# OmerMersin/video-stab

Hardware: AMD Instinct MI355X
Metric: stabilized frames/sec @1080p (whole job; warp-stage HBM GB/s in roofline) (higher is better)
Workload: dtype u8

## Files before the change

video-stab_amd/csrc/batch_schedule.cpp:

```cpp
#include <cstring>
#include <new>

#include "stab_internal.h"

using namespace vsd;

struct vs_batch {
    int device = 0, S = 0, B = 0, cap = 0;
    bool own = false;
    std::vector<vs_stab*> m;
    vs_stab* ref = nullptr;
    std::string err;
    FirstFailure failure;
    hipStream_t st = nullptr, st_pre = nullptr, st_det = nullptr, st_up = nullptr;
    bool allocated = false;
    uint8_t* h_tables = nullptr;
    size_t h_set_bytes = 0, ho_pairs = 0, ho_lk = 0, ho_rs = 0, ho_tail = 0, ho_gf = 0, ho_seg = 0;
    uint8_t* d_all = nullptr;
    uint8_t *d_lk[2] = {nullptr, nullptr}, *d_rs[2] = {nullptr, nullptr}, *d_tail[2] = {nullptr, nullptr}, *d_seg[2] = {nullptr, nullptr}, *d_gf = nullptr;
    uint8_t* d_tin[2] = {nullptr, nullptr};
    ImgPair* d_pairs[2] = {nullptr, nullptr};
    size_t up_bytes = 0;
    int pre_rel_step = -1;
    double* d_MinvB[2] = {nullptr, nullptr};
// ... 186 lines not shown

int fill_stream_items(vs_batch* g, vs_stab* s, const vs_batch::HostSet& H, const BorderPlan& bp, int ndue, int first, StepPlan& P) {
    const vs_params_c& p = s->p;
    const int ns = (int)s->bq.size(), dset = g->dev_set(P.k), set = g->pend_set;
    vs_batch::Ready& R = g->next;
    int npad = 0;
    for (int i = 0; i < ns; i++) {
        const int idx = first + i;
        const vs_stab::BFrame& b = s->bq[i];
        const vs_stab::ItemBufs& it = s->items[i];
        LKLevel L[MAX_PYR];
        fill_lk_levels(s, b.pv, b.c, L);
        const int cap = std::max(b.lk_cap, 0);
        P.n_max = std::max(P.n_max, cap);
        uint8_t *rs = H.rs + ransac_item_bytes() * idx, *tail = H.tail + tail_item_bytes() * idx;
        VS_OBJ_TRY(g, lk_fill_item(H.lk + lk_item_bytes() * idx, L, s->levels, s->d_pts[b.lk_buf], cap, s->d_npts[b.lk_buf], it.next, it.status, it.err,
                              p.lk_win_size, p.lk_max_iters, p.lk_epsilon));
        VS_OBJ_TRY(g, ransac_fill_item(rs, s->d_pts[b.lk_buf], it.next, it.status, cap, s->d_npts[b.lk_buf], it.vp, it.vc, it.m, 4, p.ransac_threshold,
                                  p.ransac_max_iters, s->tab, it.counts, it.model, it.inliers, it.info, s->d_traj, &s->tp, s->d_dbg, b.have_prev_gray));
        ransac_item_set_last(rs, i == ns - 1 ? 1 : 0);
        ransac_item_set_tail_in(rs, g->d_tin[dset] + tail_in_bytes() * idx);
        double* minv = nullptr;
        WarpTabJob jobs[2] = {{nullptr, nullptr, nullptr, 0, 0}, {nullptr, nullptr, nullptr, 0, 0}};
        if (b.out_due) {
            const int j = P.npend++;
            minv = g->d_MinvB[set] + 12 * j;
            R.srcs[j] = b.out_frame; R.dsts[j] = b.d_out; R.slots[j] = b.out_slot; R.owner[j] = s; R.pad_idx[j] = npad;
            if (P.all_apart && std::min(WARP_BATCH_MAX, ndue - j / WARP_BATCH_MAX * WARP_BATCH_MAX) >= WARP_TAB_MIN) {
                const WarpEnds e = warp_ends(s, b.out_frame, b.d_out, npad, bp);
                int32_t* T = g->d_tabs[set] + (size_t)j * g->tab_ints;
                jobs[0] = WarpTabJob{T, e.src, e.dst, bp.pw, bp.ph};
// ... 118 lines not shown
    g->last_det_batch = k;
    return VS_OK;
}

int step_issue_main(vs_batch* g, const std::vector<vs_stab*>& act, const StepPlan& P, bool warps_go, int kd) {
    const vs_stab* s0 = g->ref;
    const int dset = g->dev_set(P.k), set = g->pend_set;
    hipStream_t st = g->st;
    if (warps_go && g->last_warp_set >= 0) VS_OBJ_HIP(g, hipStreamWaitEvent(st, g->ev_warp[g->last_warp_set], 0));
    else VS_OBJ_HIP(g, hipStreamWaitEvent(st, g->ev_bpre, 0));
    for (vs_stab* s : act)
        if (s->pts_pending[0]) { VS_OBJ_HIP(g, hipStreamWaitEvent(st, s->pts_event[0], 0)); s->pts_pending[0] = false; }
    if (kd >= 0) VS_OBJ_HIP(g, hipStreamWaitEvent(st, g->det_event(kd), 0));
    {
        StageScope t(g->ref, VS_STAGE_LK, st);
        VS_OBJ_TRY(g, launch_pyr_lk_batch(g->d_lk[dset], P.n, P.n_max, s0->p.lk_win_size, st));
    }
    {
        StageScope t(g->ref, VS_STAGE_RANSAC, st);
        VS_OBJ_TRY(g, launch_ransac_score_batch(g->d_rs[dset], P.n, s0->p.ransac_max_iters, P.n_max, st));
    }
    for (vs_stab* s : act)
        if (s->dbg_delay_us > 0) { VS_OBJ_TRY(g, launch_spin(s->dbg_delay_us, st)); break; }
    if (P.npend > 0 && g->warp_valid[set]) {
        VS_OBJ_HIP(g, hipStreamWaitEvent(st, g->ev_warp[set], 0));
        g->warp_valid[set] = false;
    }
    {
        StageScope t(g->ref, VS_STAGE_TRAJ, st);
        VS_OBJ_TRY(g, launch_ransac_tail_group(g->d_rs[dset], g->d_tail[dset], g->d_seg[dset], g->d_tin[dset], P.nseg, P.max_n, P.n, P.any_apart, st));
    }
// ... 222 lines not shown
```

video-stab_amd/csrc/k_lk.hip:

```cpp
#include "vs_common.h"

namespace vsd {
namespace {

constexpr int MAX_LEVELS = 8;

struct LKArgs {
    LKLevel levels[MAX_LEVELS];
    int max_level;
    const float* prev_pts;
    float* next_pts;
    uint8_t* status;
    float* err;
    int n;
    const int32_t* d_n;
    int win;
    int max_count;
    double eps2;
};

template <int CTRL>
__device__ __forceinline__ int dpp_mov(int v) {
    return __builtin_amdgcn_update_dpp(0, v, CTRL, 0xF, 0xF, true);
}
// ... 30 lines not shown

__device__ __forceinline__ int descale(int x, int n) { return (x + (1 << (n - 1))) >> n; }

struct Weights { int w00, w01, w10, w11; };

__device__ __forceinline__ Weights make_weights(float a, float b) {
    Weights w;
    w.w00 = f_round((1.f - a) * (1.f - b) * 16384.f);
    w.w01 = f_round(a * (1.f - b) * 16384.f);
    w.w10 = f_round((1.f - a) * b * 16384.f);
    w.w11 = 16384 - w.w00 - w.w01 - w.w10;
    return w;
}

typedef const __attribute__((address_space(1))) uint8_t* gmem_u8;
__device__ __forceinline__ gmem_u8 uniform_global(const uint8_t* p) {
    const unsigned long long v = (unsigned long long)p;
    const unsigned lo = (unsigned)__builtin_amdgcn_readfirstlane((int)(unsigned)v), hi = (unsigned)__builtin_amdgcn_readfirstlane((int)(unsigned)(v >> 32));
    return (gmem_u8)(((unsigned long long)hi << 32) | lo);
}

constexpr int LK_MARGIN = 6;
constexpr int LK_WIN_MAX = 31;



__device__ __forceinline__ void divmod_small(int i, int d, float inv_d, int& q, int& r) {
    q = (int)(((float)i + 0.5f) * inv_d);
    r = i - q * d;
}

template <int NPX>
__device__ __forceinline__ void lk_track(const LKArgs& a, const int pt) {
    constexpr int WM = NPX <= 4 ? 16 : (NPX <= 7 ? 21 : LK_WIN_MAX);
    constexpr int PWM = WM + 1, RWM = WM + 1 + 2 * LK_MARGIN;
    constexpr int DR = NPX <= 7 ? 3 : 5;
    constexpr int PPM = (PWM + 2 + 3) & ~3;
    constexpr int SRM = (PWM + 1 + 3) / 4, NGM = (PWM + DR - 1) / DR;
    static_assert(SRM * NGM <= 64, "one derivative round per level");
    constexpr int PN = (PPM * (PWM + 2) + 63) / 64, RN = (RWM * RWM + 63) / 64;
    constexpr int PBYTES = (PN * 64 > PPM * (NGM * DR + 2) + 4 ? PN * 64 : PPM * (NGM * DR + 2) + 4);
    __shared__ __attribute__((aligned(16))) uint8_t pI_[4 + PBYTES];
    uint8_t* const pI = pI_ + 4;
    __shared__ __attribute__((aligned(16))) short2 pD[(PWM + 1) * PPM];
    __shared__ uint8_t region[RN * 64];
    const int lane = threadIdx.x;
    int n = a.n;
    if (a.d_n) { int dn = *a.d_n; n = dn < n ? dn : n; }
    if (pt >= n) return;
    const int win = a.win, area = win * win;
    const int PW = win + 1, PP = (PW + 2 + 3) & ~3;
    const int RW = win + 1 + 2 * LK_MARGIN;
    const float inv_pp = 1.0f / (float)PP, inv_rw = 1.0f / (float)RW, inv_win = 1.0f / (float)win;
    uint32_t off[NPX];
#pragma unroll
    for (int k = 0; k < NPX; k++) {
        const int p = lane + 64 * k;
        int yy = 0, xx = 0;
        if (p < area) divmod_small(p, win, inv_win, yy, xx);
        off[k] = (uint32_t)((yy + 1) * PP + xx + 1) | ((uint32_t)(yy * RW + xx) << 16);
    }
#define LK_VALID(k) (lane + 64 * (k) < area)
#define LK_POFF(k) ((int)(off[k] & 0xFFFFu))
#define LK_ROFF(k) ((int)(off[k] >> 16))
    int p_y0, p_x0, p_sy, p_sx, r_y0, r_x0, r_sy, r_sx;
    divmod_small(lane, PP, inv_pp, p_y0, p_x0);
    divmod_small(64, PP, inv_pp, p_sy, p_sx);
    divmod_small(lane, RW, inv_rw, r_y0, r_x0);
    divmod_small(64, RW, inv_rw, r_sy, r_sx);
    const float halfWin = (win - 1) * 0.5f;
    const float FLT_SCALE = 1.f / (1 << 20);
    const float px0 = a.prev_pts[2 * pt], py0 = a.prev_pts[2 * pt + 1];
    float outx = 0.f, outy = 0.f;
    int status = 1;
    float err = 0.f;

    for (int level = a.max_level; level >= 0; level--) {
        const LKLevel L = a.levels[level];
        const float scale = (float)(1. / (double)(1 << level));
        float prevx = px0 * scale, prevy = py0 * scale;
        if (level == a.max_level) { outx = prevx; outy = prevy; }
        else { outx = outx * 2.f; outy = outy * 2.f; }
        prevx -= halfWin; prevy -= halfWin;
        const int ipx = f_floor(prevx), ipy = f_floor(prevy);
        if (ipx < -win || ipx >= L.w || ipy < -win || ipy >= L.h) {
            if (level == 0) { status = 0; err = 0.f; }
            continue;
        }
        float cx = outx - halfWin, cy = outy - halfWin;
        int rx0 = f_floor(cx) - LK_MARGIN, ry0 = f_floor(cy) - LK_MARGIN;
        __syncthreads();
        const int pcount = PP * (PW + 2);
        if (ipx >= 1 && ipy >= 1 && ipx - 1 + PP <= L.w && ipy + PW + 1 <= L.h) {
            const gmem_u8 pbase = uniform_global(L.prev + ((size_t)(ipy - 1) * L.stride + (ipx - 1)));
            constexpr int PB_ = 10;
            int y = p_y0, x = p_x0;
#pragma unroll
            for (int k0 = 0; k0 < PN; k0 += PB_) {
                uint8_t vI[PB_];
#pragma unroll
                for (int k = k0; k < k0 + PB_ && k < PN; k++) {
                    const bool ok = lane + 64 * k < pcount;
                    vI[k - k0] = pbase[ok ? (uint32_t)(y * (int)L.stride + x) : 0u];
                    x += p_sx; y += p_sy;
                    if (x >= PP) { x -= PP; y++; }
                }
#pragma unroll
                for (int k = k0; k < k0 + PB_ && k < PN; k++) pI[lane + 64 * k] = vI[k - k0];
                __builtin_amdgcn_sched_barrier(0);
            }
        } else {
            int y = p_y0, x = p_x0;
            for (int i = lane; i < pcount; i += 64) {
                const int X = ipx - 1 + x, Y = ipy - 1 + y;
                pI[i] = L.prev[(size_t)reflect101(Y, L.h) * L.stride + reflect101(X, L.w)];
                x += p_sx; y += p_sy;
                if (x >= PP) { x -= PP; y++; }
            }
        }
        auto stage_region = [&]() {
            const bool inside = rx0 >= 0 && ry0 >= 0 && rx0 + RW <= L.w && ry0 + RW <= L.h;
            int y = r_y0, x = r_x0;
            asm volatile("" : "+v"(x), "+v"(y));
            if (inside) {
                const gmem_u8 rbase = uniform_global(L.next + ((size_t)ry0 * L.stride + rx0));
                constexpr int RB_ = 10;
#pragma unroll
                for (int k0 = 0; k0 < RN; k0 += RB_) {
                    uint8_t vR[RB_];
#pragma unroll
                    for (int k = k0; k < k0 + RB_ && k < RN; k++) {
                        const bool ok = lane + 64 * k < RW * RW;
                        vR[k - k0] = rbase[ok ? (uint32_t)(y * (int)L.stride + x) : 0u];
                        x += r_sx; y += r_sy;
                        if (x >= RW) { x -= RW; y++; }
                    }
#pragma unroll
                    for (int k = k0; k < k0 + RB_ && k < RN; k++) region[lane + 64 * k] = vR[k - k0];
                    __builtin_amdgcn_sched_barrier(0);
                }
            } else {
                for (int i = lane; i < RW * RW; i += 64) {
                    const int X = rx0 + x, Y = ry0 + y;
                    region[i] = L.next[(size_t)reflect101(Y, L.h) * L.stride + reflect101(X, L.w)];
                    x += r_sx; y += r_sy;
                    if (x >= RW) { x -= RW; y++; }
                }
            }
        };
        stage_region();
        __syncthreads();
        {
            const int sr = (PW + 1 + 3) >> 2;
            int g, c;
            divmod_small(lane, sr, 1.0f / (float)sr, g, c);
            const int y = 1 + g * DR, x = 4 * c;
            if (y <= PW) {
                const bool masked = !(ipx >= 0 && ipy >= 0 && ipx + PW <= L.w && ipy + PW <= L.h);
                int t[3][6];
                auto load_row = [&](int j, int* tj) {
                    const uint32_t* q = reinterpret_cast<const uint32_t*>(pI + j * PP) + c;
                    const uint32_t lo = q[-1], mid = q[0], hi = q[1];
                    tj[0] = lo >> 24;
                    tj[1] = mid & 255u; tj[2] = (mid >> 8) & 255u; tj[3] = (mid >> 16) & 255u; tj[4] = mid >> 24;
                    tj[5] = hi & 255u;
                };
                load_row(y - 1, t[0]);
                load_row(y, t[1]);
#pragma unroll
                for (int r = 0; r < DR; r++) {
                    const int* t0 = t[r % 3];
                    const int* t1 = t[(r + 1) % 3];
                    int* t2 = t[(r + 2) % 3];
                    load_row(y + r + 1, t2);
                    int av[6], bv[6];
#pragma unroll
                    for (int k = 0; k < 6; k++) {
                        av[k] = (t0[k] + t2[k]) * 3 + t1[k] * 10;
                        bv[k] = t2[k] - t0[k];
                    }
                    uint32_t o[4];
#pragma unroll
                    for (int k = 0; k < 4; k++) {
                        const int dx = av[k + 2] - av[k], dy = (bv[k + 2] + bv[k]) * 3 + bv[k + 1] * 10;
                        o[k] = ((uint32_t)dx & 0xFFFFu) | ((uint32_t)dy << 16);
                        if (masked && ((unsigned)(ipx - 1 + x + k) >= (unsigned)L.w || (unsigned)(ipy - 1 + y + r) >= (unsigned)L.h)) o[k] = 0u;
                    }
                    if (y + r <= PW) *reinterpret_cast<uint4*>(&pD[(y + r) * PP + x]) = make_uint4(o[0], o[1], o[2], o[3]);
                    __builtin_amdgcn_sched_barrier(0);
                }
            }
        }
        __syncthreads();
#pragma unroll
        for (int k = 0; k < NPX; k++) asm volatile("" : "+v"(off[k]));
        Weights wt = make_weights(prevx - ipx, prevy - ipy);
        short Iw[NPX], Ix[NPX], Iy[NPX];
        int pA11 = 0, pA12 = 0, pA22 = 0;
#pragma unroll
        for (int k = 0; k < NPX; k++) {
            const int o = LK_POFF(k);
            int ival = descale(__mul24((int)pI[o], wt.w00) + __mul24((int)pI[o + 1], wt.w01) +
                               __mul24((int)pI[o + PP], wt.w10) + __mul24((int)pI[o + PP + 1], wt.w11), 9);
            const short2 d00 = pD[o], d01 = pD[o + 1], d10 = pD[o + PP], d11 = pD[o + PP + 1];
            int ixval = descale(__mul24((int)d00.x, wt.w00) + __mul24((int)d01.x, wt.w01) +
                                __mul24((int)d10.x, wt.w10) + __mul24((int)d11.x, wt.w11), 14);
            int iyval = descale(__mul24((int)d00.y, wt.w00) + __mul24((int)d01.y, wt.w01) +
                                __mul24((int)d10.y, wt.w10) + __mul24((int)d11.y, wt.w11), 14);
            if (!LK_VALID(k)) { ival = 0; ixval = 0; iyval = 0; }
            Iw[k] = (short)ival; Ix[k] = (short)ixval; Iy[k] = (short)iyval;
            pA11 += __mul24(ixval, ixval);
            pA12 += __mul24(ixval, iyval);
            pA22 += __mul24(iyval, iyval);
        }
        const long long sA11 = wave_sum(pA11), sA12 = wave_sum(pA12), sA22 = wave_sum(pA22);
        const float A11 = (float)sA11 * FLT_SCALE, A12 = (float)sA12 * FLT_SCALE, A22 = (float)sA22 * FLT_SCALE;
// ... 11 lines not shown
            if (inx < -win || inx >= L.w || iny < -win || iny >= L.h) {
                if (level == 0) status = 0;
                break;
            }
            wt = make_weights(cx - inx, cy - iny);
            int lx = inx - rx0, ly = iny - ry0;
            if (!(lx >= 0 && ly >= 0 && lx + win + 1 <= RW && ly + win + 1 <= RW)) {
                __syncthreads();
                rx0 = inx - LK_MARGIN; ry0 = iny - LK_MARGIN;
                stage_region();
                __syncthreads();
                lx = LK_MARGIN; ly = LK_MARGIN;
            }
            int pb1 = 0, pb2 = 0;
            {
                const int rbase = ly * RW + lx;
#pragma unroll
                for (int k = 0; k < NPX; k++) {
                    const uint8_t* r0 = &region[rbase + LK_ROFF(k)];
                    const int v = descale(__mul24((int)r0[0], wt.w00) + __mul24((int)r0[1], wt.w01) +
                                          __mul24((int)r0[RW], wt.w10) + __mul24((int)r0[RW + 1], wt.w11), 9);
                    const int diff = v - Iw[k];
                    pb1 += __mul24(diff, (int)Ix[k]);
                    pb2 += __mul24(diff, (int)Iy[k]);
                }
            }
            const long long sb1 = wave_sum(pb1), sb2 = wave_sum(pb2);
            const float b1 = (float)sb1 * FLT_SCALE, b2 = (float)sb2 * FLT_SCALE;
            const float dx = (A12 * b2 - A22 * b1) * D;
            const float dy = (A12 * b1 - A11 * b2) * D;
            cx += dx; cy += dy;
            outx = cx + halfWin; outy = cy + halfWin;
            if ((double)dx * (double)dx + (double)dy * (double)dy <= a.eps2) break;
            if (j > 0 && (double)fabsf(dx + pdx) < 0.01 && (double)fabsf(dy + pdy) < 0.01) {
                outx -= dx * 0.5f; outy -= dy * 0.5f;
                break;
            }
            pdx = dx; pdy = dy;
        }
        if (status && level == 0) {
            const float npx = outx - halfWin, npy = outy - halfWin;
            const int inx = f_floor(npx), iny = f_floor(npy);
            if (inx < -win || inx >= L.w || iny < -win || iny >= L.h) {
                status = 0;
            } else {
                wt = make_weights(npx - inx, npy - iny);
                int lx = inx - rx0, ly = iny - ry0;
                if (!(lx >= 0 && ly >= 0 && lx + win + 1 <= RW && ly + win + 1 <= RW)) {
                    __syncthreads();
                    rx0 = inx - LK_MARGIN; ry0 = iny - LK_MARGIN;
                    stage_region();
                    __syncthreads();
                    lx = LK_MARGIN; ly = LK_MARGIN;
                }
                int es = 0;
                {
                    const int rbase = ly * RW + lx;
#pragma unroll
                    for (int k = 0; k < NPX; k++) {
                        const uint8_t* r0 = &region[rbase + LK_ROFF(k)];
                        const int v = descale(__mul24((int)r0[0], wt.w00) + __mul24((int)r0[1], wt.w01) +
                                              __mul24((int)r0[RW], wt.w10) + __mul24((int)r0[RW + 1], wt.w11), 9);
                        const int diff = v - Iw[k];
                        es += LK_VALID(k) ? (diff < 0 ? -diff : diff) : 0;
                    }
                }
                const long long est = wave_sum(es);
                err = (float)est * 1.f / (float)(32 * win * win);
            }
        }
    }
#undef LK_VALID
#undef LK_POFF
#undef LK_ROFF
    if (lane == 0) {
        a.next_pts[2 * pt] = outx;
        a.next_pts[2 * pt + 1] = outy;
        a.status[pt] = (uint8_t)status;
        a.err[pt] = err;
    }
}

template <int NPX>
__global__ __launch_bounds__(64) void lk_kernel(LKArgs a) { lk_track<NPX>(a, blockIdx.x); }

template <int NPX>
__global__ __launch_bounds__(64) void lk_batch_kernel(const LKArgs* __restrict__ table) {
    lk_track<NPX>(table[blockIdx.y], blockIdx.x);
}

int fill_lk_args(LKArgs& a, const LKLevel* levels, int max_level, const float* d_prev_pts, int n, const int32_t* d_n,
                 float* d_next_pts, uint8_t* d_status, float* d_err, int win, int max_iters, double eps) {
    if (!levels || max_level < 0 || max_level >= MAX_LEVELS || n < 0 || win < 3 || win > 31 ||
        !d_prev_pts || !d_next_pts || !d_status || !d_err) {
        set_last_error("pyr_lk: invalid argument (3 <= win <= 31, max_level < 8)");
        return VS_ERR_INVALID_ARG;
    }
    for (int i = 0; i <= max_level; i++) a.levels[i] = levels[i];
    for (int i = max_level + 1; i < MAX_LEVELS; i++) a.levels[i] = levels[max_level];
    a.max_level = max_level;
    a.prev_pts = d_prev_pts; a.next_pts = d_next_pts; a.status = d_status; a.err = d_err;
    a.n = n; a.d_n = d_n; a.win = win;
    a.max_count = max_iters < 0 ? 0 : (max_iters > 100 ? 100 : max_iters);
    double e = eps < 0 ? 0. : (eps > 10. ? 10. : eps);
    a.eps2 = e * e;
    return VS_OK;
}

}

size_t lk_item_bytes() { return sizeof(LKArgs); }

int lk_fill_item(void* host_item, const LKLevel* levels, int max_level, const float* d_prev_pts, int n,
                 const int32_t* d_n, float* d_next_pts, uint8_t* d_status, float* d_err, int win, int max_iters,
                 double eps) {
    return fill_lk_args(*static_cast<LKArgs*>(host_item), levels, max_level, d_prev_pts, n, d_n, d_next_pts, d_status,
                        d_err, win, max_iters, eps);
}

int launch_pyr_lk_batch(const void* d_table, int items, int n_max, int win, hipStream_t st) {
    if (!d_table || items < 1 || items > 65535 || n_max < 0 || win < 3 || win > 31) {
        set_last_error("pyr_lk_batch: invalid argument");
        return VS_ERR_INVALID_ARG;
    }
    if (n_max == 0) return VS_OK;
    const LKArgs* t = static_cast<const LKArgs*>(d_table);
    const int npx = (win * win + 63) / 64;
    dim3 grid(n_max, items), block(64);
    if (npx <= 4) hipLaunchKernelGGL(lk_batch_kernel<4>, grid, block, 0, st, t);
    else if (npx <= 7) hipLaunchKernelGGL(lk_batch_kernel<7>, grid, block, 0, st, t);
    else hipLaunchKernelGGL(lk_batch_kernel<16>, grid, block, 0, st, t);
    VS_HIP_TRY(hipGetLastError());
    return VS_OK;
}

int launch_pyr_lk(const LKLevel* levels, int max_level, const float* d_prev_pts, int n,
                  const int32_t* d_n, float* d_next_pts, uint8_t* d_status, float* d_err, int win,
                  int max_iters, double eps, hipStream_t st) {
    LKArgs a;
    VS_TRY(fill_lk_args(a, levels, max_level, d_prev_pts, n, d_n, d_next_pts, d_status, d_err, win, max_iters, eps));
    if (n == 0) return VS_OK;
    const int npx = (win * win + 63) / 64;
    dim3 grid(n), block(64);
    if (npx <= 4) hipLaunchKernelGGL(lk_kernel<4>, grid, block, 0, st, a);
    else if (npx <= 7) hipLaunchKernelGGL(lk_kernel<7>, grid, block, 0, st, a);
    else hipLaunchKernelGGL(lk_kernel<16>, grid, block, 0, st, a);
    VS_HIP_TRY(hipGetLastError());
    return VS_OK;
}

int run_pyr_lk_op(const uint8_t* d_prev, const uint8_t* d_next, size_t stride, int w, int h,
                  const float* d_prev_pts, int n, float* d_next_pts, uint8_t* d_status,
                  float* d_err, int win, int max_level, int max_iters, double eps, hipStream_t st) {
    if (!d_prev || !d_next || w <= 0 || h <= 0 || max_level < 0 || max_level >= MAX_LEVELS) {
        set_last_error("pyr_lk: invalid argument");
        return VS_ERR_INVALID_ARG;
    }
    int lw[MAX_LEVELS], lh[MAX_LEVELS];
    int levels = 0;
    {
        int sw = w, sh = h;
// ... 34 lines not shown
```

video-stab_amd/csrc/launchers.h:

```cpp
#ifndef VS_LAUNCHERS_H
#define VS_LAUNCHERS_H

#include "traj_state.h"
#include "vs_common.h"
#include "warp_tab.h"

namespace vsd {

struct RansacTables;
int get_ransac_tables(int max_m, int iters, const RansacTables** out);
int launch_ransac(const float* d_from, const float* d_to, const uint8_t* d_status, int n, const int32_t* d_n, float* d_vp, float* d_vc, int32_t* d_m,
                  int min_points, double thr, int iters, const RansacTables* tab, int32_t* d_counts, double* d_model, uint8_t* d_inliers,
                  int32_t* d_info, TrajState* traj, const TrajParams* tp, vs_debug_frame* dbg, int have_prev_gray, hipStream_t st);
size_t ransac_item_bytes();
int ransac_fill_item(void* host_item, const float* d_from, const float* d_to, const uint8_t* d_status, int n, const int32_t* d_n, float* d_vp,
                     float* d_vc, int32_t* d_m, int min_points, double thr, int iters, const RansacTables* tab, int32_t* d_counts, double* d_model,
                     uint8_t* d_inliers, int32_t* d_info, TrajState* traj, const TrajParams* tp, vs_debug_frame* dbg, int have_prev_gray);
void ransac_item_set_tail_in(void* host_item, void* d_tail_in);
void ransac_item_set_last(void* host_item, int last);
int launch_ransac_score_batch(const void* d_table, int items, int iters, int n_max, hipStream_t st);
size_t tail_item_bytes();
void tail_fill_item(void* host_item, int out_due, int out_idx, double* d_Minv_out, const WarpTabJob* tabs);
void tail_item_set_seg(void* host_item, int seg);
size_t tail_in_bytes();
size_t tail_seg_bytes();
void tail_fill_seg(void* host_seg, int first, int n, float* d_M_out, TrajState* traj, vs_debug_frame* dbg, int smoothing_method);
int launch_ransac_tail_group(const void* d_table, const void* d_tail, const void* d_segs, const void* d_tail_in, int nsegs, int max_n, int items,
                             int any_apart, hipStream_t st);

size_t lk_item_bytes();
int lk_fill_item(void* host_item, const LKLevel* levels, int max_level, const float* d_prev_pts, int n, const int32_t* d_n, float* d_next_pts,
                 uint8_t* d_status, float* d_err, int win, int max_iters, double eps);
int launch_pyr_lk_batch(const void* d_table, int items, int n_max, int win, hipStream_t st);
size_t gftt_item_bytes();
int gftt_fill_item(void* host_item, const uint8_t* d_gray, size_t stride, int w, int h, int max_corners, double quality, double min_distance,
                   int block_size, const GfttWork& wk, float* d_pts, int32_t* d_count);
int launch_gftt_batch(const void* d_table, int items, int w, int h, int block_size, hipStream_t st, int what);

int launch_traj_emit(TrajState* s, const TrajParams& p, int idx, float* M_out, double* Minv_out, vs_debug_frame* dbg, hipStream_t st,
                     float* t_out = nullptr);
int launch_traj_reset(TrajState* s, int smoothing_radius, hipStream_t st);
int launch_spin(int microseconds, hipStream_t st);
int launch_fade_blend(const uint8_t* d_hist, uint8_t* d_frame, size_t bytes, float alpha, float beta, hipStream_t st);
int launch_fade_update(uint8_t* d_hist, const uint8_t* d_stab, size_t sstride, int row_bytes, int rows, hipStream_t st);
int launch_make_border(const uint8_t* src, size_t sstride, int w, int h, int cn, uint8_t* dst, size_t dstride, int b, int border, hipStream_t st);
int launch_resize_linear(const uint8_t* d_src, size_t sstride, int sw, int sh, int cn, uint8_t* d_dst, size_t dstride, int dw, int dh, hipStream_t st);

}
// ... 2 lines not shown
```

video-stab_amd/csrc/stab_internal.h:

```cpp
#ifndef VS_STAB_INTERNAL_H
#define VS_STAB_INTERNAL_H

#include <algorithm>
#include <deque>
#include <initializer_list>
#include <memory>
#include <vector>

#include "canvas.h"
#include "host_helper.h"
#include "launchers.h"

namespace vsd {

constexpr int FRAME_RING = 128;
constexpr int FRAME_RING_MAX = 192;
constexpr int MAX_PYR = 8;
constexpr int NPYR = 3;
constexpr int BATCH_MAX = 64;
constexpr int EVR = 4;

struct Pyramid {
    uint8_t* img[MAX_PYR] = {};
};
// ... 42 lines not shown
    int last_out_w = 0, last_out_h = 0;
    int orig_w = 0, orig_h = 0;
    int host_radius = 30;
    int dbg_delay_us = 0;
    uint8_t* d_first_gray = nullptr;
    std::vector<vsd::Pyramid> pyr;
    int npyr = vsd::NPYR;
    bool prev_small = false;
    bool have_prev_gray = false;
    int ncap = 0;
    std::vector<float*> d_pts;
    std::vector<int32_t*> d_npts;
    std::vector<int> pts_cap;
    int pp = 0;
    int last_lk_pp = 0;
    float *d_next = nullptr, *d_err = nullptr, *d_vp = nullptr, *d_vc = nullptr;
    uint8_t *d_status = nullptr, *d_inliers = nullptr;
    int32_t *d_m = nullptr, *d_info = nullptr, *d_counts = nullptr;
    double* d_model = nullptr;
    void* d_gftt_scratch = nullptr;
    vsd::GfttWork gw;
    const vsd::RansacTables* tab = nullptr;
    vsd::TrajState* d_traj = nullptr;
    vsd::TrajParams tp;
    float* d_M = nullptr;
    double* d_Minv = nullptr;
    vs_debug_frame* d_dbg = nullptr;
    int last_detect_pp = -1;
    bool last_detected = false;
    int last_gray_buf = 0;
    uint8_t* d_tmp = nullptr;
// ... 33 lines not shown
    hipEvent_t ev_emit = nullptr, ev_warp[2] = {nullptr, nullptr};
    bool warp_valid[2] = {false, false};
    int batch = 1;
    bool batch_active = false;
    struct BFrame {
        int f, c, pv;
        const uint8_t* frame; bool prev_small;
        bool detect; int det_buf;
        int lk_buf, lk_cap;
        bool out_due; int out_slot, out_idx; const uint8_t* out_frame; uint8_t* d_out; size_t out_stride;
        int have_prev_gray;
    };
    std::vector<BFrame> bq;
    int kp_cur = 0, kp_next = 1;
    std::vector<vsd::GfttWork> gws;
    struct ItemBufs { float *next, *err, *vp, *vc; uint8_t *status, *inliers; int32_t *m, *info, *counts; double* model; };
    std::vector<ItemBufs> items;
    const float* dbg_prev_pts = nullptr; const float* dbg_next = nullptr;
    const uint8_t *dbg_status = nullptr, *dbg_inliers = nullptr;
    const float* dbg_det_pts = nullptr; const int32_t* dbg_det_n = nullptr;
    const int32_t* dbg_gftt_counters = nullptr;
    int prof_mode = 0;
    struct Pending { hipEvent_t a, b; int stage; };
    std::vector<Pending> pending;
    std::vector<hipEvent_t> ev_pool;
};

namespace vsd {

struct StageScope {
    vs_stab* s;
// ... 90 lines not shown
```

video-stab_amd/csrc/stabilizer.cpp:

```cpp
#include <array>
#include <cstring>
#include <cstdlib>
#include <map>
#include <mutex>
#include <new>

#include "stab_internal.h"

using namespace vsd;

namespace {

int fmt_cn(int fmt) {
    switch (fmt) {
        case VS_FMT_BGR8: case VS_FMT_RGB8: return 3;
        case VS_FMT_BGRA8: case VS_FMT_RGBA8: return 4;
        case VS_FMT_NV12: case VS_FMT_GRAY8: return 1;
        case VS_FMT_P010: return 2;
        default: return 0;
    }
}

int effective_radius(int r) { return std::max(5, std::min(r, 35)); }
int flush_warps(vs_stab* s);
// ... 94 lines not shown
        s->group = s->own;
    }
    s->free_slots.clear();
    s->ring_frames = (s->batch_active && B > 32) ? FRAME_RING_MAX : FRAME_RING;
    for (int i = 0; i < s->ring_frames; i++) { s->free_slots.push_back(i); s->slot_valid[i] = false; }
    s->ncap = std::max(s->p.max_corners, 1);
    const int ncap = s->ncap;
    size_t off = 0;
    auto take = [&](size_t bytes) { size_t o = off; off += (bytes + 255) & ~(size_t)255; return o; };
    size_t o_first = take((size_t)480 * 270);
    std::vector<std::array<size_t, MAX_PYR>> o_img(s->npyr);
    for (int k = 0; k < s->npyr; k++)
        for (int l = 0; l <= s->levels; l++) o_img[k][l] = take((size_t)s->lw[l] * s->lh[l]);
    std::vector<size_t> o_pts(nkp), o_npts(nkp);
    for (int k = 0; k < nkp; k++) { o_pts[k] = take((size_t)ncap * 8); o_npts[k] = take(16); }
    struct ItemOff { size_t next, err, vp, vc, status, inl, m, info, counts, model; };
    std::vector<ItemOff> o_it(B);
    for (int k = 0; k < B; k++) {
        o_it[k].next = take((size_t)ncap * 8); o_it[k].err = take((size_t)ncap * 4);
        o_it[k].vp = take((size_t)ncap * 8); o_it[k].vc = take((size_t)ncap * 8);
        o_it[k].status = take(ncap); o_it[k].inl = take(ncap);
        o_it[k].m = take(16); o_it[k].info = take(16); o_it[k].counts = take((size_t)s->p.ransac_max_iters * 4);
        o_it[k].model = take(48);
    }
    size_t o_traj = take(sizeof(TrajState)), o_M = take(96), o_Minv = take(96), o_dbg = take(sizeof(vs_debug_frame));
    size_t o_MinvB[2] = {take((size_t)BATCH_MAX * 96), take((size_t)BATCH_MAX * 96)};
    int tow, toh;
    out_size(s, w, h, &tow, &toh);
    const size_t o_tabs = take(warp_tabs_ints(std::max(w, tow), std::max(h, toh), WARP_BATCH_MAX) * sizeof(int32_t));
    VS_OBJ_HIP(s, hipMalloc((void**)&s->d_all, off));
    VS_OBJ_HIP(s, hipMemsetAsync(s->d_all, 0, off, s->st));
    uint8_t* b = s->d_all;
    s->d_first_gray = b + o_first;
    for (int k = 0; k < s->npyr; k++)
        for (int l = 0; l <= s->levels; l++) s->pyr[k].img[l] = b + o_img[k][l];
    for (int k = 0; k < nkp; k++) { s->d_pts[k] = (float*)(b + o_pts[k]); s->d_npts[k] = (int32_t*)(b + o_npts[k]); }
    for (int k = 0; k < B; k++) {
        vs_stab::ItemBufs& it = s->items[k];
        it.next = (float*)(b + o_it[k].next); it.err = (float*)(b + o_it[k].err);
        it.vp = (float*)(b + o_it[k].vp); it.vc = (float*)(b + o_it[k].vc);
        it.status = b + o_it[k].status; it.inliers = b + o_it[k].inl;
        it.m = (int32_t*)(b + o_it[k].m); it.info = (int32_t*)(b + o_it[k].info); it.counts = (int32_t*)(b + o_it[k].counts);
        it.model = (double*)(b + o_it[k].model);
    }
    s->d_next = s->items[0].next; s->d_err = s->items[0].err; s->d_vp = s->items[0].vp; s->d_vc = s->items[0].vc;
    s->d_status = s->items[0].status; s->d_inliers = s->items[0].inliers;
    s->d_m = s->items[0].m; s->d_info = s->items[0].info; s->d_counts = s->items[0].counts; s->d_model = s->items[0].model;
    s->d_traj = (TrajState*)(b + o_traj);
    s->d_M = (float*)(b + o_M); s->d_Minv = (double*)(b + o_Minv); s->d_dbg = (vs_debug_frame*)(b + o_dbg);
    s->d_MinvB[0] = (double*)(b + o_MinvB[0]); s->d_MinvB[1] = (double*)(b + o_MinvB[1]);
    s->d_tabs_def = (int32_t*)(b + o_tabs);
    s->pend.clear(); s->pend_set = 0; s->warp_valid[0] = s->warp_valid[1] = false;
    const int gmaxw = std::max(s->aw, 480), gmaxh = std::max(s->ah, 270);
    const int cap = gmaxw * gmaxh / 4 + 64;
    const size_t gwb = (gftt_work_bytes(gmaxw, gmaxh, cap) + 255) & ~(size_t)255;
    VS_OBJ_HIP(s, hipMalloc(&s->d_gftt_scratch, gwb * ngw));
    s->gws.assign(ngw, GfttWork());
    for (int k = 0; k < ngw; k++) gftt_work_carve((uint8_t*)s->d_gftt_scratch + gwb * k, gmaxw, gmaxh, cap, &s->gws[k]);
    s->gw = s->gws[0];
    s->dbg_gftt_counters = s->gw.counters;
// ... 104 lines not shown
        s->last_detect_pp = q;
        s->dbg_det_pts = s->d_pts[q]; s->dbg_det_n = s->d_npts[q];
        s->counters.detections++;
    }

    VS_OBJ_HIP(s, hipStreamWaitEvent(s->st, s->ev_pre[c], 0));
    if (s->pts_pending[pp]) {
        VS_OBJ_HIP(s, hipStreamWaitEvent(s->st, s->pts_event[pp], 0));
        s->pts_pending[pp] = false;
    }
    LKLevel L[MAX_PYR];
    fill_lk_levels(s, pv, c, L);
    const int cap = s->pts_cap[pp];
    {
        StageScope t(s, VS_STAGE_LK, s->st);
        VS_OBJ_TRY(s, launch_pyr_lk(L, s->levels, s->d_pts[pp], cap, s->d_npts[pp], s->d_next, s->d_status, s->d_err,
                               p.lk_win_size, p.lk_max_iters, p.lk_epsilon, s->st));
    }
    s->last_lk_pp = pp;
    if (s->dbg_delay_us > 0) VS_OBJ_TRY(s, launch_spin(s->dbg_delay_us, s->st));
    {
        StageScope t(s, VS_STAGE_RANSAC, s->st);
        VS_OBJ_TRY(s, launch_ransac(s->d_pts[pp], s->d_next, s->d_status, std::max(cap, 0), s->d_npts[pp], s->d_vp, s->d_vc,
                               s->d_m, 4, p.ransac_threshold, p.ransac_max_iters, s->tab, s->d_counts, s->d_model,
                               s->d_inliers, s->d_info, s->d_traj, &s->tp, s->d_dbg, s->have_prev_gray ? 1 : 0, s->st));
    }
    VS_OBJ_HIP(s, hipEventRecord(s->ev_lk[f % EVR], s->st));
    s->dbg_prev_pts = s->d_pts[pp]; s->dbg_next = s->d_next; s->dbg_status = s->d_status; s->dbg_inliers = s->d_inliers;
    s->n_transforms++;
    s->pp = next_pp;
    s->last_gray_buf = c;
// ... 764 lines not shown
```

Measured before the change: 129,600.

## Stage LK patches with dword loads and drop unused error computation

The LK tracker now stages the prev patch and the next-frame region into shared memory with 32-bit global loads from a 4-byte-aligned base, padding row pitches and carrying a sub-dword shift into the indexing, instead of byte loads. It also adds an ERR template flag so callers that never consume the per-point error skip the final error pass and the write, and the err buffers are removed. This cuts global load instruction count and some arithmetic in the LK stage. In exchange, rows are wider, shared memory grows, and the indexing is more complex, with fallback paths for unaligned or border cases.

```diff
diff --git a/video-stab_amd/csrc/batch_schedule.cpp b/video-stab_amd/csrc/batch_schedule.cpp
--- a/video-stab_amd/csrc/batch_schedule.cpp
+++ b/video-stab_amd/csrc/batch_schedule.cpp
@@ -224,7 +224,7 @@
         const int cap = std::max(b.lk_cap, 0);
         P.n_max = std::max(P.n_max, cap);
         uint8_t *rs = H.rs + ransac_item_bytes() * idx, *tail = H.tail + tail_item_bytes() * idx;
-        VS_OBJ_TRY(g, lk_fill_item(H.lk + lk_item_bytes() * idx, L, s->levels, s->d_pts[b.lk_buf], cap, s->d_npts[b.lk_buf], it.next, it.status, it.err,
+        VS_OBJ_TRY(g, lk_fill_item(H.lk + lk_item_bytes() * idx, L, s->levels, s->d_pts[b.lk_buf], cap, s->d_npts[b.lk_buf], it.next, it.status, nullptr,
                               p.lk_win_size, p.lk_max_iters, p.lk_epsilon));
         VS_OBJ_TRY(g, ransac_fill_item(rs, s->d_pts[b.lk_buf], it.next, it.status, cap, s->d_npts[b.lk_buf], it.vp, it.vc, it.m, 4, p.ransac_threshold,
                                   p.ransac_max_iters, s->tab, it.counts, it.model, it.inliers, it.info, s->d_traj, &s->tp, s->d_dbg, b.have_prev_gray));
@@ -373,7 +373,7 @@
     if (kd >= 0) VS_OBJ_HIP(g, hipStreamWaitEvent(st, g->det_event(kd), 0));
     {
         StageScope t(g->ref, VS_STAGE_LK, st);
-        VS_OBJ_TRY(g, launch_pyr_lk_batch(g->d_lk[dset], P.n, P.n_max, s0->p.lk_win_size, st));
+        VS_OBJ_TRY(g, launch_pyr_lk_batch(g->d_lk[dset], P.n, P.n_max, s0->p.lk_win_size, false, st));
     }
     {
         StageScope t(g->ref, VS_STAGE_RANSAC, st);
diff --git a/video-stab_amd/csrc/k_lk.hip b/video-stab_amd/csrc/k_lk.hip
--- a/video-stab_amd/csrc/k_lk.hip
+++ b/video-stab_amd/csrc/k_lk.hip
@@ -68,6 +68,7 @@
 }
 
 typedef const __attribute__((address_space(1))) uint8_t* gmem_u8;
+typedef const __attribute__((address_space(1))) uint32_t* gmem_u32;
 __device__ __forceinline__ gmem_u8 uniform_global(const uint8_t* p) {
     const unsigned long long v = (unsigned long long)p;
     const unsigned lo = (unsigned)__builtin_amdgcn_readfirstlane((int)(unsigned)v), hi = (unsigned)__builtin_amdgcn_readfirstlane((int)(unsigned)(v >> 32));
@@ -84,44 +85,46 @@
     r = i - q * d;
 }
 
-template <int NPX>
+template <int NPX, bool ERR>
 __device__ __forceinline__ void lk_track(const LKArgs& a, const int pt) {
     constexpr int WM = NPX <= 4 ? 16 : (NPX <= 7 ? 21 : LK_WIN_MAX);
     constexpr int PWM = WM + 1, RWM = WM + 1 + 2 * LK_MARGIN;
     constexpr int DR = NPX <= 7 ? 3 : 5;
-    constexpr int PPM = (PWM + 2 + 3) & ~3;
-    constexpr int SRM = (PWM + 1 + 3) / 4, NGM = (PWM + DR - 1) / DR;
+    constexpr int PPM = ((PWM + 2 + 3) & ~3) + 4;
+    constexpr int SRM = (PWM + 3) / 4 + 1, NGM = (PWM + DR - 1) / DR;
     static_assert(SRM * NGM <= 64, "one derivative round per level");
-    constexpr int PN = (PPM * (PWM + 2) + 63) / 64, RN = (RWM * RWM + 63) / 64;
-    constexpr int PBYTES = (PN * 64 > PPM * (NGM * DR + 2) + 4 ? PN * 64 : PPM * (NGM * DR + 2) + 4);
+    constexpr int RPM = (RWM + 3 + 3) & ~3;
+    constexpr int PN = (PPM / 4 * (PWM + 2) + 63) / 64, RN = (RPM / 4 * RWM + 63) / 64;
+    constexpr int PBYTES = (PN * 256 > PPM * (NGM * DR + 2) + 4 ? PN * 256 : PPM * (NGM * DR + 2) + 4);
     __shared__ __attribute__((aligned(16))) uint8_t pI_[4 + PBYTES];
     uint8_t* const pI = pI_ + 4;
     __shared__ __attribute__((aligned(16))) short2 pD[(PWM + 1) * PPM];
-    __shared__ uint8_t region[RN * 64];
+    __shared__ __attribute__((aligned(16))) uint8_t region[RN * 256];
     const int lane = threadIdx.x;
     int n = a.n;
     if (a.d_n) { int dn = *a.d_n; n = dn < n ? dn : n; }
     if (pt >= n) return;
     const int win = a.win, area = win * win;
-    const int PW = win + 1, PP = (PW + 2 + 3) & ~3;
-    const int RW = win + 1 + 2 * LK_MARGIN;
-    const float inv_pp = 1.0f / (float)PP, inv_rw = 1.0f / (float)RW, inv_win = 1.0f / (float)win;
+    const int PW = win + 1, PP = ((PW + 2 + 3) & ~3) + 4;
+    const int RW = win + 1 + 2 * LK_MARGIN, RP = (RW + 3 + 3) & ~3;
+    const int PQ = PP >> 2, RQ = RP >> 2;
+    const float inv_pq = 1.0f / (float)PQ, inv_rq = 1.0f / (float)RQ, inv_win = 1.0f / (float)win;
     uint32_t off[NPX];
 #pragma unroll
     for (int k = 0; k < NPX; k++) {
         const int p = lane + 64 * k;
         int yy = 0, xx = 0;
         if (p < area) divmod_small(p, win, inv_win, yy, xx);
-        off[k] = (uint32_t)((yy + 1) * PP + xx + 1) | ((uint32_t)(yy * RW + xx) << 16);
+        off[k] = (uint32_t)((yy + 1) * PP + xx + 1) | ((uint32_t)(yy * RP + xx) << 16);
     }
 #define LK_VALID(k) (lane + 64 * (k) < area)
 #define LK_POFF(k) ((int)(off[k] & 0xFFFFu))
 #define LK_ROFF(k) ((int)(off[k] >> 16))
     int p_y0, p_x0, p_sy, p_sx, r_y0, r_x0, r_sy, r_sx;
-    divmod_small(lane, PP, inv_pp, p_y0, p_x0);
-    divmod_small(64, PP, inv_pp, p_sy, p_sx);
-    divmod_small(lane, RW, inv_rw, r_y0, r_x0);
-    divmod_small(64, RW, inv_rw, r_sy, r_sx);
+    divmod_small(lane, PQ, inv_pq, p_y0, p_x0);
+    divmod_small(64, PQ, inv_pq, p_sy, p_sx);
+    divmod_small(lane, RQ, inv_rq, r_y0, r_x0);
+    divmod_small(64, RQ, inv_rq, r_sy, r_sx);
     const float halfWin = (win - 1) * 0.5f;
     const float FLT_SCALE = 1.f / (1 << 20);
     const float px0 = a.prev_pts[2 * pt], py0 = a.prev_pts[2 * pt + 1];
@@ -144,70 +147,118 @@
         float cx = outx - halfWin, cy = outy - halfWin;
         int rx0 = f_floor(cx) - LK_MARGIN, ry0 = f_floor(cy) - LK_MARGIN;
         __syncthreads();
-        const int pcount = PP * (PW + 2);
-        if (ipx >= 1 && ipy >= 1 && ipx - 1 + PP <= L.w && ipy + PW + 1 <= L.h) {
-            const gmem_u8 pbase = uniform_global(L.prev + ((size_t)(ipy - 1) * L.stride + (ipx - 1)));
-            constexpr int PB_ = 10;
+        const bool dwords = (((size_t)L.prev | (size_t)L.next | L.stride) & 3) == 0;
+        const bool prows = ipy >= 1 && ipy + PW + 1 <= L.h;
+        int sp = 0;
+        if (dwords && prows && ipx >= 1 && ((ipx - 1) & ~3) + PP <= L.w) {
+            sp = (ipx - 1) & 3;
+            const gmem_u32 pbase = (gmem_u32)uniform_global(L.prev + ((size_t)(ipy - 1) * L.stride + (size_t)((ipx - 1) & ~3)));
+            const int pcount = PQ * (PW + 2), q = (int)(L.stride >> 2);
             int y = p_y0, x = p_x0;
-#pragma unroll
-            for (int k0 = 0; k0 < PN; k0 += PB_) {
-                uint8_t vI[PB_];
-#pragma unroll
-                for (int k = k0; k < k0 + PB_ && k < PN; k++) {
-                    const bool ok = lane + 64 * k < pcount;
-                    vI[k - k0] = pbase[ok ? (uint32_t)(y * (int)L.stride + x) : 0u];
-                    x += p_sx; y += p_sy;
+            uint32_t vI[PN];
+#pragma unroll
+            for (int k = 0; k < PN; k++) {
+                const bool ok = lane + 64 * k < pcount;
+                vI[k] = pbase[ok ? (uint32_t)(y * q + x) : 0u];
+                x += p_sx; y += p_sy;
+                if (x >= PQ) { x -= PQ; y++; }
+            }
+#pragma unroll
+            for (int k = 0; k < PN; k++) reinterpret_cast<uint32_t*>(pI)[lane + 64 * k] = vI[k];
+            __builtin_amdgcn_sched_barrier(0);
+        } else {
+            const int pcount = PP * (PW + 2);
+            const float inv_pp = 1.0f / (float)PP;
+            int y, x, sy, sx;
+            divmod_small(lane, PP, inv_pp, y, x);
+            divmod_small(64, PP, inv_pp, sy, sx);
+            asm volatile("" : "+v"(x), "+v"(y));
+            if (prows && ipx >= 1 && ipx - 1 + PP <= L.w) {
+                const gmem_u8 pbase = uniform_global(L.prev + ((size_t)(ipy - 1) * L.stride + (ipx - 1)));
+                constexpr int PNB = (PPM * (PWM + 2) + 63) / 64, PB_ = 10;
+#pragma unroll
+                for (int k0 = 0; k0 < PNB; k0 += PB_) {
+                    uint8_t vI[PB_];
+#pragma unroll
+                    for (int k = k0; k < k0 + PB_ && k < PNB; k++) {
+                        const bool ok = lane + 64 * k < pcount;
+                        vI[k - k0] = pbase[ok ? (uint32_t)(y * (int)L.stride + x) : 0u];
+                        x += sx; y += sy;
+                        if (x >= PP) { x -= PP; y++; }
+                    }
+#pragma unroll
+                    for (int k = k0; k < k0 + PB_ && k < PNB; k++) pI[lane + 64 * k] = vI[k - k0];
+                    __builtin_amdgcn_sched_barrier(0);
+                }
+            } else {
+                for (int i = lane; i < pcount; i += 64) {
+                    const int X = ipx - 1 + x, Y = ipy - 1 + y;
+                    pI[i] = L.prev[(size_t)reflect101(Y, L.h) * L.stride + reflect101(X, L.w)];
+                    x += sx; y += sy;
                     if (x >= PP) { x -= PP; y++; }
                 }
-#pragma unroll
-                for (int k = k0; k < k0 + PB_ && k < PN; k++) pI[lane + 64 * k] = vI[k - k0];
+            }
+        }
+        int sr = 0;
+        auto stage_region = [&]() {
+            const bool rrows = ry0 >= 0 && ry0 + RW <= L.h;
+            if (dwords && rrows && rx0 >= 0 && (rx0 & ~3) + RP <= L.w) {
+                sr = rx0 & 3;
+                const gmem_u32 rbase = (gmem_u32)uniform_global(L.next + ((size_t)ry0 * L.stride + (size_t)(rx0 & ~3)));
+                const int q = (int)(L.stride >> 2);
+                int y = r_y0, x = r_x0;
+                asm volatile("" : "+v"(x), "+v"(y));
+                uint32_t vR[RN];
+#pragma unroll
+                for (int k = 0; k < RN; k++) {
+                    const bool ok = lane + 64 * k < RQ * RW;
+                    vR[k] = rbase[ok ? (uint32_t)(y * q + x) : 0u];
+                    x += r_sx; y += r_sy;
+                    if (x >= RQ) { x -= RQ; y++; }
+                }
+#pragma unroll
+                for (int k = 0; k < RN; k++) reinterpret_cast<uint32_t*>(region)[lane + 64 * k] = vR[k];
                 __builtin_amdgcn_sched_barrier(0);
-            }
-        } else {
-            int y = p_y0, x = p_x0;
-            for (int i = lane; i < pcount; i += 64) {
-                const int X = ipx - 1 + x, Y = ipy - 1 + y;
-                pI[i] = L.prev[(size_t)reflect101(Y, L.h) * L.stride + reflect101(X, L.w)];
-                x += p_sx; y += p_sy;
-                if (x >= PP) { x -= PP; y++; }
-            }
-        }
-        auto stage_region = [&]() {
-            const bool inside = rx0 >= 0 && ry0 >= 0 && rx0 + RW <= L.w && ry0 + RW <= L.h;
-            int y = r_y0, x = r_x0;
+                return;
+            }
+            sr = 0;
+            const float inv_rp = 1.0f / (float)RP;
+            int y, x, sy, sx;
+            divmod_small(lane, RP, inv_rp, y, x);
+            divmod_small(64, RP, inv_rp, sy, sx);
             asm volatile("" : "+v"(x), "+v"(y));
-            if (inside) {
+            if (rrows && rx0 >= 0 && rx0 + RP <= L.w) {
                 const gmem_u8 rbase = uniform_global(L.next + ((size_t)ry0 * L.stride + rx0));
-                constexpr int RB_ = 10;
-#pragma unroll
-                for (int k0 = 0; k0 < RN; k0 += RB_) {
+                constexpr int RNB = (RPM * RWM + 63) / 64, RB_ = 10;
+#pragma unroll
+                for (int k0 = 0; k0 < RNB; k0 += RB_) {
                     uint8_t vR[RB_];
 #pragma unroll
-                    for (int k = k0; k < k0 + RB_ && k < RN; k++) {
-                        const bool ok = lane + 64 * k < RW * RW;
+                    for (int k = k0; k < k0 + RB_ && k < RNB; k++) {
+                        const bool ok = lane + 64 * k < RP * RW;
                         vR[k - k0] = rbase[ok ? (uint32_t)(y * (int)L.stride + x) : 0u];
-                        x += r_sx; y += r_sy;
-                        if (x >= RW) { x -= RW; y++; }
+                        x += sx; y += sy;
+                        if (x >= RP) { x -= RP; y++; }
                     }
 #pragma unroll
-                    for (int k = k0; k < k0 + RB_ && k < RN; k++) region[lane + 64 * k] = vR[k - k0];
+                    for (int k = k0; k < k0 + RB_ && k < RNB; k++) region[lane + 64 * k] = vR[k - k0];
                     __builtin_amdgcn_sched_barrier(0);
                 }
             } else {
-                for (int i = lane; i < RW * RW; i += 64) {
+                for (int i = lane; i < RP * RW; i += 64) {
                     const int X = rx0 + x, Y = ry0 + y;
                     region[i] = L.next[(size_t)reflect101(Y, L.h) * L.stride + reflect101(X, L.w)];
-                    x += r_sx; y += r_sy;
-                    if (x >= RW) { x -= RW; y++; }
+                    x += sx; y += sy;
+                    if (x >= RP) { x -= RP; y++; }
                 }
             }
         };
         stage_region();
         __syncthreads();
         {
-            const int sr = (PW + 1 + 3) >> 2;
+            const int ns = ((PW + 3) >> 2) + 1;
             int g, c;
-            divmod_small(lane, sr, 1.0f / (float)sr, g, c);
+            divmod_small(lane, ns, 1.0f / (float)ns, g, c);
             const int y = 1 + g * DR, x = 4 * c;
             if (y <= PW) {
                 const bool masked = !(ipx >= 0 && ipy >= 0 && ipx + PW <= L.w && ipy + PW <= L.h);
@@ -238,7 +289,7 @@
                     for (int k = 0; k < 4; k++) {
                         const int dx = av[k + 2] - av[k], dy = (bv[k + 2] + bv[k]) * 3 + bv[k + 1] * 10;
                         o[k] = ((uint32_t)dx & 0xFFFFu) | ((uint32_t)dy << 16);
-                        if (masked && ((unsigned)(ipx - 1 + x + k) >= (unsigned)L.w || (unsigned)(ipy - 1 + y + r) >= (unsigned)L.h)) o[k] = 0u;
+                        if (masked && ((unsigned)(ipx - 1 - sp + x + k) >= (unsigned)L.w || (unsigned)(ipy - 1 + y + r) >= (unsigned)L.h)) o[k] = 0u;
                     }
                     if (y + r <= PW) *reinterpret_cast<uint4*>(&pD[(y + r) * PP + x]) = make_uint4(o[0], o[1], o[2], o[3]);
                     __builtin_amdgcn_sched_barrier(0);
@@ -253,7 +304,7 @@
         int pA11 = 0, pA12 = 0, pA22 = 0;
 #pragma unroll
         for (int k = 0; k < NPX; k++) {
-            const int o = LK_POFF(k);
+            const int o = LK_POFF(k) + sp;
             int ival = descale(__mul24((int)pI[o], wt.w00) + __mul24((int)pI[o + 1], wt.w01) +
                                __mul24((int)pI[o + PP], wt.w10) + __mul24((int)pI[o + PP + 1], wt.w11), 9);
             const short2 d00 = pD[o], d01 = pD[o + 1], d10 = pD[o + PP], d11 = pD[o + PP + 1];
@@ -295,12 +346,12 @@
             }
             int pb1 = 0, pb2 = 0;
             {
-                const int rbase = ly * RW + lx;
+                const int rbase = ly * RP + lx + sr;
 #pragma unroll
                 for (int k = 0; k < NPX; k++) {
                     const uint8_t* r0 = &region[rbase + LK_ROFF(k)];
                     const int v = descale(__mul24((int)r0[0], wt.w00) + __mul24((int)r0[1], wt.w01) +
-                                          __mul24((int)r0[RW], wt.w10) + __mul24((int)r0[RW + 1], wt.w11), 9);
+                                          __mul24((int)r0[RP], wt.w10) + __mul24((int)r0[RP + 1], wt.w11), 9);
                     const int diff = v - Iw[k];
                     pb1 += __mul24(diff, (int)Ix[k]);
                     pb2 += __mul24(diff, (int)Iy[k]);
@@ -324,7 +375,7 @@
             const int inx = f_floor(npx), iny = f_floor(npy);
             if (inx < -win || inx >= L.w || iny < -win || iny >= L.h) {
                 status = 0;
-            } else {
+            } else if (ERR) {
                 wt = make_weights(npx - inx, npy - iny);
                 int lx = inx - rx0, ly = iny - ry0;
                 if (!(lx >= 0 && ly >= 0 && lx + win + 1 <= RW && ly + win + 1 <= RW)) {
@@ -336,12 +387,12 @@
                 }
                 int es = 0;
                 {
-                    const int rbase = ly * RW + lx;
+                    const int rbase = ly * RP + lx + sr;
 #pragma unroll
                     for (int k = 0; k < NPX; k++) {
                         const uint8_t* r0 = &region[rbase + LK_ROFF(k)];
                         const int v = descale(__mul24((int)r0[0], wt.w00) + __mul24((int)r0[1], wt.w01) +
-                                              __mul24((int)r0[RW], wt.w10) + __mul24((int)r0[RW + 1], wt.w11), 9);
+                                              __mul24((int)r0[RP], wt.w10) + __mul24((int)r0[RP + 1], wt.w11), 9);
                         const int diff = v - Iw[k];
                         es += LK_VALID(k) ? (diff < 0 ? -diff : diff) : 0;
                     }
@@ -358,22 +409,37 @@
         a.next_pts[2 * pt] = outx;
         a.next_pts[2 * pt + 1] = outy;
         a.status[pt] = (uint8_t)status;
-        a.err[pt] = err;
-    }
-}
-
-template <int NPX>
-__global__ __launch_bounds__(64) void lk_kernel(LKArgs a) { lk_track<NPX>(a, blockIdx.x); }
-
-template <int NPX>
+        if (ERR) a.err[pt] = err;
+    }
+}
+
+template <int NPX, bool ERR>
+__global__ __launch_bounds__(64) void lk_kernel(LKArgs a) { lk_track<NPX, ERR>(a, blockIdx.x); }
+
+template <int NPX, bool ERR>
 __global__ __launch_bounds__(64) void lk_batch_kernel(const LKArgs* __restrict__ table) {
-    lk_track<NPX>(table[blockIdx.y], blockIdx.x);
+    lk_track<NPX, ERR>(table[blockIdx.y], blockIdx.x);
+}
+
+template <bool ERR>
+void launch_lk(const LKArgs& a, dim3 grid, hipStream_t st) {
+    const int npx = (a.win * a.win + 63) / 64;
+    if (npx <= 4) hipLaunchKernelGGL((lk_kernel<4, ERR>), grid, dim3(64), 0, st, a);
+    else if (npx <= 7) hipLaunchKernelGGL((lk_kernel<7, ERR>), grid, dim3(64), 0, st, a);
+    else hipLaunchKernelGGL((lk_kernel<16, ERR>), grid, dim3(64), 0, st, a);
+}
+template <bool ERR>
+void launch_lk_batch(const LKArgs* t, int win, dim3 grid, hipStream_t st) {
+    const int npx = (win * win + 63) / 64;
+    if (npx <= 4) hipLaunchKernelGGL((lk_batch_kernel<4, ERR>), grid, dim3(64), 0, st, t);
+    else if (npx <= 7) hipLaunchKernelGGL((lk_batch_kernel<7, ERR>), grid, dim3(64), 0, st, t);
+    else hipLaunchKernelGGL((lk_batch_kernel<16, ERR>), grid, dim3(64), 0, st, t);
 }
 
 int fill_lk_args(LKArgs& a, const LKLevel* levels, int max_level, const float* d_prev_pts, int n, const int32_t* d_n,
                  float* d_next_pts, uint8_t* d_status, float* d_err, int win, int max_iters, double eps) {
     if (!levels || max_level < 0 || max_level >= MAX_LEVELS || n < 0 || win < 3 || win > 31 ||
-        !d_prev_pts || !d_next_pts || !d_status || !d_err) {
+        !d_prev_pts || !d_next_pts || !d_status) {
         set_last_error("pyr_lk: invalid argument (3 <= win <= 31, max_level < 8)");
         return VS_ERR_INVALID_ARG;
     }
@@ -399,18 +465,15 @@
                         d_err, win, max_iters, eps);
 }
 
-int launch_pyr_lk_batch(const void* d_table, int items, int n_max, int win, hipStream_t st) {
+int launch_pyr_lk_batch(const void* d_table, int items, int n_max, int win, bool want_err, hipStream_t st) {
     if (!d_table || items < 1 || items > 65535 || n_max < 0 || win < 3 || win > 31) {
         set_last_error("pyr_lk_batch: invalid argument");
         return VS_ERR_INVALID_ARG;
     }
     if (n_max == 0) return VS_OK;
     const LKArgs* t = static_cast<const LKArgs*>(d_table);
-    const int npx = (win * win + 63) / 64;
-    dim3 grid(n_max, items), block(64);
-    if (npx <= 4) hipLaunchKernelGGL(lk_batch_kernel<4>, grid, block, 0, st, t);
-    else if (npx <= 7) hipLaunchKernelGGL(lk_batch_kernel<7>, grid, block, 0, st, t);
-    else hipLaunchKernelGGL(lk_batch_kernel<16>, grid, block, 0, st, t);
+    if (want_err) launch_lk_batch<true>(t, win, dim3(n_max, items), st);
+    else launch_lk_batch<false>(t, win, dim3(n_max, items), st);
     VS_HIP_TRY(hipGetLastError());
     return VS_OK;
 }
@@ -421,11 +484,8 @@
     LKArgs a;
     VS_TRY(fill_lk_args(a, levels, max_level, d_prev_pts, n, d_n, d_next_pts, d_status, d_err, win, max_iters, eps));
     if (n == 0) return VS_OK;
-    const int npx = (win * win + 63) / 64;
-    dim3 grid(n), block(64);
-    if (npx <= 4) hipLaunchKernelGGL(lk_kernel<4>, grid, block, 0, st, a);
-    else if (npx <= 7) hipLaunchKernelGGL(lk_kernel<7>, grid, block, 0, st, a);
-    else hipLaunchKernelGGL(lk_kernel<16>, grid, block, 0, st, a);
+    if (d_err) launch_lk<true>(a, dim3(n), st);
+    else launch_lk<false>(a, dim3(n), st);
     VS_HIP_TRY(hipGetLastError());
     return VS_OK;
 }
diff --git a/video-stab_amd/csrc/launchers.h b/video-stab_amd/csrc/launchers.h
--- a/video-stab_amd/csrc/launchers.h
+++ b/video-stab_amd/csrc/launchers.h
@@ -31,7 +31,7 @@
 size_t lk_item_bytes();
 int lk_fill_item(void* host_item, const LKLevel* levels, int max_level, const float* d_prev_pts, int n, const int32_t* d_n, float* d_next_pts,
                  uint8_t* d_status, float* d_err, int win, int max_iters, double eps);
-int launch_pyr_lk_batch(const void* d_table, int items, int n_max, int win, hipStream_t st);
+int launch_pyr_lk_batch(const void* d_table, int items, int n_max, int win, bool want_err, hipStream_t st);
 size_t gftt_item_bytes();
 int gftt_fill_item(void* host_item, const uint8_t* d_gray, size_t stride, int w, int h, int max_corners, double quality, double min_distance,
                    int block_size, const GfttWork& wk, float* d_pts, int32_t* d_count);
diff --git a/video-stab_amd/csrc/stab_internal.h b/video-stab_amd/csrc/stab_internal.h
--- a/video-stab_amd/csrc/stab_internal.h
+++ b/video-stab_amd/csrc/stab_internal.h
@@ -80,7 +80,7 @@
     std::vector<int> pts_cap;
     int pp = 0;
     int last_lk_pp = 0;
-    float *d_next = nullptr, *d_err = nullptr, *d_vp = nullptr, *d_vc = nullptr;
+    float *d_next = nullptr, *d_vp = nullptr, *d_vc = nullptr;
     uint8_t *d_status = nullptr, *d_inliers = nullptr;
     int32_t *d_m = nullptr, *d_info = nullptr, *d_counts = nullptr;
     double* d_model = nullptr;
@@ -144,7 +144,7 @@
     std::vector<BFrame> bq;
     int kp_cur = 0, kp_next = 1;
     std::vector<vsd::GfttWork> gws;
-    struct ItemBufs { float *next, *err, *vp, *vc; uint8_t *status, *inliers; int32_t *m, *info, *counts; double* model; };
+    struct ItemBufs { float *next, *vp, *vc; uint8_t *status, *inliers; int32_t *m, *info, *counts; double* model; };
     std::vector<ItemBufs> items;
     const float* dbg_prev_pts = nullptr; const float* dbg_next = nullptr;
     const uint8_t *dbg_status = nullptr, *dbg_inliers = nullptr;
diff --git a/video-stab_amd/csrc/stabilizer.cpp b/video-stab_amd/csrc/stabilizer.cpp
--- a/video-stab_amd/csrc/stabilizer.cpp
+++ b/video-stab_amd/csrc/stabilizer.cpp
@@ -132,10 +132,10 @@
         for (int l = 0; l <= s->levels; l++) o_img[k][l] = take((size_t)s->lw[l] * s->lh[l]);
     std::vector<size_t> o_pts(nkp), o_npts(nkp);
     for (int k = 0; k < nkp; k++) { o_pts[k] = take((size_t)ncap * 8); o_npts[k] = take(16); }
-    struct ItemOff { size_t next, err, vp, vc, status, inl, m, info, counts, model; };
+    struct ItemOff { size_t next, vp, vc, status, inl, m, info, counts, model; };
     std::vector<ItemOff> o_it(B);
     for (int k = 0; k < B; k++) {
-        o_it[k].next = take((size_t)ncap * 8); o_it[k].err = take((size_t)ncap * 4);
+        o_it[k].next = take((size_t)ncap * 8);
         o_it[k].vp = take((size_t)ncap * 8); o_it[k].vc = take((size_t)ncap * 8);
         o_it[k].status = take(ncap); o_it[k].inl = take(ncap);
         o_it[k].m = take(16); o_it[k].info = take(16); o_it[k].counts = take((size_t)s->p.ransac_max_iters * 4);
@@ -155,13 +155,13 @@
     for (int k = 0; k < nkp; k++) { s->d_pts[k] = (float*)(b + o_pts[k]); s->d_npts[k] = (int32_t*)(b + o_npts[k]); }
     for (int k = 0; k < B; k++) {
         vs_stab::ItemBufs& it = s->items[k];
-        it.next = (float*)(b + o_it[k].next); it.err = (float*)(b + o_it[k].err);
+        it.next = (float*)(b + o_it[k].next);
         it.vp = (float*)(b + o_it[k].vp); it.vc = (float*)(b + o_it[k].vc);
         it.status = b + o_it[k].status; it.inliers = b + o_it[k].inl;
         it.m = (int32_t*)(b + o_it[k].m); it.info = (int32_t*)(b + o_it[k].info); it.counts = (int32_t*)(b + o_it[k].counts);
         it.model = (double*)(b + o_it[k].model);
     }
-    s->d_next = s->items[0].next; s->d_err = s->items[0].err; s->d_vp = s->items[0].vp; s->d_vc = s->items[0].vc;
+    s->d_next = s->items[0].next; s->d_vp = s->items[0].vp; s->d_vc = s->items[0].vc;
     s->d_status = s->items[0].status; s->d_inliers = s->items[0].inliers;
     s->d_m = s->items[0].m; s->d_info = s->items[0].info; s->d_counts = s->items[0].counts; s->d_model = s->items[0].model;
     s->d_traj = (TrajState*)(b + o_traj);
@@ -296,7 +296,7 @@
     const int cap = s->pts_cap[pp];
     {
         StageScope t(s, VS_STAGE_LK, s->st);
-        VS_OBJ_TRY(s, launch_pyr_lk(L, s->levels, s->d_pts[pp], cap, s->d_npts[pp], s->d_next, s->d_status, s->d_err,
+        VS_OBJ_TRY(s, launch_pyr_lk(L, s->levels, s->d_pts[pp], cap, s->d_npts[pp], s->d_next, s->d_status, nullptr,
                                p.lk_win_size, p.lk_max_iters, p.lk_epsilon, s->st));
     }
     s->last_lk_pp = pp;
```

Result: no change. 129,800 (median of 3 runs) (+0.2%).
